# BuzzLord/godot-audio-spatializer

Hardware: AMD Instinct MI355X
Metric: mixed AudioFrames/s (higher is better)
Workload: dtype f32

## Files before the change

godot-audio-spatializer_amd/csrc/k_hrtf_multi.hip:

```cpp
#include "gas_hrtf_wave.h"

namespace {

constexpr int MW = 8;
constexpr int MAXB = GAS_HRTF_MULTI_MAX_BLOCKS;

template <int SQ>
struct MultiLds {
	static constexpr int SLICES_F2 = MW * LDS_F2_HALF;
	static constexpr int FD_F2 = MW * 2 * 512;
	static constexpr int TOTAL_F2 = SLICES_F2 + FD_F2;
	static constexpr int HL = (8 - SQ) * 64;
	static constexpr int LEFT_BYTES = 160 * 1024 - TOTAL_F2 * 8 - 1024 * 8 - 64;
	static constexpr int HIST_ROWS = LEFT_BYTES / (MW * HL * 4);
};

__device__ __forceinline__ void lds_wait_at_least(const uint32_t *flag, uint32_t want) {
	while (__atomic_load_n(flag, __ATOMIC_RELAXED) < want) {
		__builtin_amdgcn_s_sleep(1);
	}
	__builtin_amdgcn_fence(__ATOMIC_ACQUIRE, "workgroup");
}

template <int SQ, bool HIST_LDS>
__global__ __launch_bounds__(MW * 64, GAS_HRTF_WAVES_PER_SIMD) void k_hrtf_multi(gas_group_args g, gas_hrtf_blocks mb, const uint32_t *__restrict__ peak_bits, uint32_t peak_all, gas_dev_state st, gas_hrtf_table tab, const float2 *__restrict__ tw, float *__restrict__ partials) {
	constexpr int FQ = 2 * SQ;
	constexpr int HQ = 8 - SQ;
	constexpr int NQ = 8 + SQ;
	constexpr uint32_t F = FQ * 64;
	constexpr uint32_t HL = HQ * 64;
	__shared__ float2 lds_all[MultiLds<SQ>::TOTAL_F2];
	__shared__ float2 tw_lds[1024];
	__shared__ float hist_lds[HIST_LDS ? MW * MultiLds<SQ>::HIST_ROWS * HL : 4];
	__shared__ uint32_t arrived, consumed;
	const int lane = threadIdx.x & 63;
	const int wave = __builtin_amdgcn_readfirstlane(threadIdx.x >> 6);
	float2 *lds = lds_all + wave * LDS_F2_HALF;
	float *my_hist = hist_lds + (HIST_LDS ? wave * MultiLds<SQ>::HIST_ROWS * HL : 0);
	float2 *fd = lds_all + MultiLds<SQ>::SLICES_F2;
	const uint32_t K = mb.k;

	const float4 tw_in = reinterpret_cast<const float4 *>(tw)[threadIdx.x & 511];
	if (threadIdx.x == 0) {
		arrived = 0;
		consumed = 0;
	}
	uint32_t first, last;
	wave_range(g.n, blockIdx.x * MW + wave, gridDim.x * MW, first, last);
	const uint32_t cnt = last - first;
	const bool have = (uint32_t)lane < cnt;
	uint32_t my_slot = 0, my_row = 0, my_dir = 0, my_flag = 0;
	float my_g0 = 0.0f, my_g1 = 0.0f;
	if (have) {
		const uint32_t e = first + lane;
		my_slot = g.slots ? g.slots[e] : g.slot_base + e;
		my_row = g.rows ? g.rows[e] : e;
	}
	gas_audio_frame raw[FQ];
	float rawh[HQ];
	if (cnt > 0) {
		const uint32_t s0 = (uint32_t)__builtin_amdgcn_readlane((int)my_slot, 0), r0 = (uint32_t)__builtin_amdgcn_readlane((int)my_row, 0);
		if constexpr (HIST_LDS) {
			constexpr int HR = MultiLds<SQ>::HIST_ROWS;
			float stage[HR][HQ];
#pragma unroll
			for (int r = 0; r < HR; r++) {
				if ((uint32_t)r < cnt) {
					const uint32_t sr = (uint32_t)__builtin_amdgcn_readlane((int)my_slot, r);
					load_history<HQ>(st.hrtf_hist + (size_t)sr * HL, lane, stage[r]);
				}
			}
#pragma unroll
			for (int r = 0; r < HR; r++) {
				if ((uint32_t)r < cnt) {
					store_history<HQ>(my_hist + (size_t)r * HL, lane, stage[r]);
				}
			}
		} else {
			load_history<HQ>(st.hrtf_hist + (size_t)s0 * HL, lane, rawh);
		}
#pragma unroll
		for (int q = 0; q < FQ; q++) {
			raw[q] = (GAS_ABL & 8) ? gas_audio_frame{ (float)lane, (float)r0 } : nt_load_frame(mb.src[0] + (size_t)r0 * F + lane + 64 * q);
		}
	}
	auto block_params = [&](uint32_t b, float keep_g, uint32_t keep_d, float &g1, uint32_t &d) {
		const gas_params *fr = mb.fresh[b];
		g1 = keep_g;
		d = keep_d;
		if (have && (fr || b == 0)) {
			const gas_params *P = fr ? fr + my_row : st.params + my_slot;
			const float2 gd = *reinterpret_cast<const float2 *>(&P->hrtf_gain);
			const uint32_t dd = __float_as_uint(gd.y);
			g1 = gd.x;
			d = dd < tab.dirs ? dd : 0;
		}
	};
	if (have) {
		my_g0 = st.hrtf_prev_gain[my_slot];
		const uint32_t e = first + lane;
		my_flag = peak_all ? 1u : (peak_bits ? (peak_bits[e >> 5] >> (e & 31)) & 1u : 0u);
	}
	block_params(0, 0.0f, 0, my_g1, my_dir);
	if (threadIdx.x < 512) {
		reinterpret_cast<float4 *>(tw_lds)[threadIdx.x] = tw_in;
	}
	__syncthreads();
	float2 t1[8], t2[8];
#pragma unroll
	for (int k = 0; k < 8; k++) {
		t1[k] = tw_lds[k * 64 + lane];
		t2[k] = tw_lds[(8 + k) * 64 + lane];
	}
	const float lane_f = (float)lane;

	for (uint32_t b = 0; b < K; b++) {
		float *peaks_b = mb.peaks[b];
		const gas_audio_frame *src_b = mb.src[b];
		const gas_audio_frame *src_wrap = mb.src[b + 1 < K ? b + 1 : b];
		float2 aYL[8], aYR[8], zp[8];
		float4 hs[8];
#pragma unroll
		for (int j = 0; j < 8; j++) {
			aYL[j] = make_float2(0.0f, 0.0f);
			aYR[j] = make_float2(0.0f, 0.0f);
			zp[j] = make_float2(0.0f, 0.0f);
		}
		float nx_g1 = my_g1;
		uint32_t nx_dir = my_dir;
		if (b + 1 < K) {
			block_params(b + 1, my_g1, my_dir, nx_g1, nx_dir);
		}
		bool have_prev = false;
		uint32_t prev_flag = 0, prev_row = 0;
		auto products = [&](bool more, uint32_t next_dir) {
			float2 yl[8], yr[8];
			if (have_prev) {
				finish_spectra(lane, hs);
#pragma unroll
				for (int j = 0; j < 8; j++) {
					cmac_fixed(aYL[j], zp[j], hs[j].x, hs[j].y);
					cmac_fixed(aYR[j], zp[j], hs[j].z, hs[j].w);
				}
				if (prev_flag) {
#pragma unroll
					for (int j = 0; j < 8; j++) {
						yl[j] = cmul_fixed(zp[j], hs[j].x, hs[j].y);
						yr[j] = cmul_fixed(zp[j], hs[j].z, hs[j].w);
					}
				}
			}
			if (more) {
				issue_spectra(tab.spec, next_dir, lane, hs);
			}
			if (have_prev && prev_flag) {
				fft512<true>(yl, t1, t2, lds, lane);
				fft512<true>(yr, t1, t2, lds, lane);
				float pkl = 0.0f, pkr = 0.0f;
#pragma unroll
				for (int t = 0; t < SQ; t++) {
					pkl = fmaxf(pkl, fmaxf(fabsf(yl[HQ + t].x), fabsf(yl[HQ + t].y)));
					pkr = fmaxf(pkr, fmaxf(fabsf(yr[HQ + t].x), fabsf(yr[HQ + t].y)));
				}
				pkl = wave_max(pkl);
				pkr = wave_max(pkr);
				if (lane == 0) {
					peaks_b[(size_t)prev_row * 2] = pkl;
					peaks_b[(size_t)prev_row * 2 + 1] = pkr;
				}
			}
		};

		for (uint32_t i = 0; i < cnt; i++) {
			const uint32_t slot = (uint32_t)__builtin_amdgcn_readlane((int)my_slot, (int)i);
			const uint32_t row = (uint32_t)__builtin_amdgcn_readlane((int)my_row, (int)i);
			const uint32_t dir = (uint32_t)__builtin_amdgcn_readlane((int)my_dir, (int)i);
			const float g0 = __int_as_float(__builtin_amdgcn_readlane(__float_as_int(my_g0), (int)i));
			const float g1 = __int_as_float(__builtin_amdgcn_readlane(__float_as_int(my_g1), (int)i));
			const uint32_t flag = (uint32_t)__builtin_amdgcn_readlane((int)my_flag, (int)i);
			float xq[NQ];
			if constexpr (HIST_LDS) {
				load_history<HQ>(my_hist + (size_t)i * HL, lane, rawh);
			}
#pragma unroll
			for (int q = 0; q < HQ; q++) {
				xq[q] = rawh[q];
			}
			if constexpr (!HIST_LDS) {
#pragma unroll
				for (int q = 0; q < hrtf_dead_regs<SQ>(); q++) {
					asm volatile("" ::"v"(rawh[q]));
				}
			}
			float lf = lane_f;
			asm volatile("" : "+v"(lf));
#pragma unroll
			for (int q = 0; q < hrtf_unkept_regs<SQ>(); q++) {
				const float mono = (raw[q].left + raw[q].right) * 0.5f;
				const float t = (lf + (float)(64 * q)) * (1.0f / (float)F);
				xq[HQ + q] = window_sample(mono, ramp_weight(g0, g1, t, 1 - t));
			}
#pragma unroll
			for (int q = hrtf_unkept_regs<SQ>(); q < FQ; q++) {
				const float mono = (raw[q].left + raw[q].right) * 0.5f;
				const float t = (lf + (float)(64 * q)) * (1.0f / (float)F);
				xq[HQ + q] = window_sample_kept(mono, ramp_weight(g0, g1, t, 1 - t));
			}
			if (!HIST_LDS || b + 1 == K) {
				store_history<HQ>(st.hrtf_hist + (size_t)slot * HL, lane, &xq[FQ]);
			} else {
				store_history<HQ>(my_hist + (size_t)i * HL, lane, &xq[FQ]);
			}
			const bool wrap = i + 1 == cnt;
			{
				const uint32_t ni = wrap ? 0u : i + 1;
				const uint32_t nrow = (uint32_t)__builtin_amdgcn_readlane((int)my_row, (int)ni);
				const gas_audio_frame *nsrc = (wrap ? src_wrap : src_b) + (size_t)nrow * F;
				if constexpr (!HIST_LDS) {
					const uint32_t nslot = (uint32_t)__builtin_amdgcn_readlane((int)my_slot, (int)ni);
					load_history<HQ>(st.hrtf_hist + (size_t)nslot * HL, lane, rawh);
				}
#pragma unroll
				for (int q = 0; q < FQ; q++) {
					raw[q] = (GAS_ABL & 8) ? gas_audio_frame{ (float)lane, (float)nrow } : nt_load_frame(nsrc + lane + 64 * q);
				}
			}
			float2 zs[8];
#pragma unroll
			for (int j = 0; j < 8; j++) {
				zs[j] = hrtf_window_z<SQ>(xq, j);
			}
			fft512<false>(zs, t1, t2, lds, lane);
			products(true, dir);
#pragma unroll
			for (int j = 0; j < 8; j++) {
				zp[j] = zs[j];
			}
			have_prev = true;
			prev_flag = flag;
			prev_row = row;
		}
		const int ep0 = (int)(2 * (b & 3));
		const gas_deferred_reduce job = mb.job[b];
		float4 jr[JOB_ROWS];
		const uint32_t jw = (uint32_t)((wave - ep0 - 2) & 7), jx = blockIdx.x & 7, ji = blockIdx.x >> 3;
		const uint32_t job_col = (((ji >> 1) * 8 + jx) * 8) + (ji & 1) * 4 + jw;
		const bool job_mine = job.partials != nullptr && jw < GAS_HRTF_JOB_WAVES && job_col < job.elems / 4;
		products(false, 0);

		lds_wait_at_least(&consumed, 2 * b);
#pragma unroll
		for (int j = 0; j < 8; j++) {
			fd[(wave * 2 + 0) * 512 + j * 64 + lane] = aYL[j];
			fd[(wave * 2 + 1) * 512 + j * 64 + lane] = aYR[j];
		}
		__builtin_amdgcn_fence(__ATOMIC_RELEASE, "workgroup");
		if (lane == 0) {
			__atomic_fetch_add(&arrived, 1u, __ATOMIC_RELAXED);
		}
		if (job_mine) {
			job_issue(job, job_col, lane, jr);
			job_finish(job, job_col, lane, jr);
		}
		if (wave == ep0 || wave == ep0 + 1) {
			const int ear = wave - ep0;
			lds_wait_at_least(&arrived, MW * (b + 1));
			float2 y[8];
#pragma unroll
			for (int j = 0; j < 8; j++) {
				y[j] = fd[ear * 512 + j * 64 + lane];
			}
#pragma unroll
			for (int w = 1; w < MW; w++) {
#pragma unroll
				for (int j = 0; j < 8; j++) {
					y[j] = cadd(y[j], fd[(w * 2 + ear) * 512 + j * 64 + lane]);
				}
			}
			__builtin_amdgcn_fence(__ATOMIC_RELEASE, "workgroup");
			if (lane == 0) {
				__atomic_fetch_add(&consumed, 1u, __ATOMIC_RELAXED);
			}
			fft512<true>(y, t1, t2, lds, lane);
			float *my_partial = partials + ((size_t)mb.p_offset[b] + blockIdx.x) * (size_t)(F * 2);
#pragma unroll
			for (int t = 0; t < SQ; t++) {
				const int fa = lane + 64 * t, fb = lane + 64 * (SQ + t);
				my_partial[fa * 2 + ear] = y[HQ + t].x;
				my_partial[fb * 2 + ear] = y[HQ + t].y;
			}
		}
		if (have && !my_flag) {
			*reinterpret_cast<float2 *>(peaks_b + (size_t)my_row * 2) = make_float2(__builtin_inff(), __builtin_inff());
		}
		my_g0 = my_g1;
		my_g1 = nx_g1;
		my_dir = nx_dir;
	}

	if (have) {
		st.hrtf_prev_gain[my_slot] = my_g0;
		if (mb.last_fresh) {
			const float4 *src4 = reinterpret_cast<const float4 *>(mb.last_fresh + my_row);
			float4 *dst4 = reinterpret_cast<float4 *>(st.params + my_slot);
#pragma unroll
			for (int k = 0; k < 8; k++) {
				dst4[k] = src4[k];
			}
		}
	}
}

}

bool gas_hrtf_multi_hist_in_lds(uint32_t n, uint32_t frames) {
	const uint32_t wgs = gas_hrtf_uni_partials(n);
	const uint32_t per_wave = (n + wgs * MW - 1) / (wgs * MW);
	switch (frames / 128) {
		case 1:
			return per_wave <= (uint32_t)MultiLds<1>::HIST_ROWS;
		case 2:
			return per_wave <= (uint32_t)MultiLds<2>::HIST_ROWS;
		case 3:
			return per_wave <= (uint32_t)MultiLds<3>::HIST_ROWS;
		default:
			return per_wave <= (uint32_t)MultiLds<4>::HIST_ROWS;
	}
}

hipError_t gas_launch_hrtf_multi(hipStream_t stream, const gas_group_args &g, const gas_hrtf_blocks &mb, const uint32_t *peak_bits, bool peak_all, const gas_dev_state &st, const gas_hrtf_table &tab, const float2 *twiddles, uint32_t frames, uint32_t hist_len, float *partials) {
	if (g.n == 0 || mb.k == 0) {
		return hipSuccess;
	}
	const uint32_t wgs = gas_hrtf_uni_partials(g.n);
	if (frames % 128 != 0 || frames > 512 || hist_len != 512 - frames / 2 || g.order != nullptr || mb.k > (uint32_t)MAXB || g.n < wgs * MW || g.n > wgs * MW * 64 || gas_hrtf_uni_waves() != (uint32_t)MW) {
		return hipErrorInvalidValue;
	}
	dim3 grid(wgs), block(MW * 64);
	const uint32_t all = peak_all ? 1u : 0u;
	const uint32_t per_wave = (g.n + wgs * MW - 1) / (wgs * MW);
#define GAS_MULTI_CASE(SQv)                                                                                                                     \
	case SQv:                                                                                                                                   \
		if (per_wave <= (uint32_t)MultiLds<SQv>::HIST_ROWS) {                                                                                   \
			hipLaunchKernelGGL((k_hrtf_multi<SQv, true>), grid, block, 0, stream, g, mb, peak_bits, all, st, tab, twiddles, partials);          \
		} else {                                                                                                                                \
			hipLaunchKernelGGL((k_hrtf_multi<SQv, false>), grid, block, 0, stream, g, mb, peak_bits, all, st, tab, twiddles, partials);         \
		}                                                                                                                                       \
		break;
	switch (frames / 128) {
		GAS_MULTI_CASE(1)
		GAS_MULTI_CASE(2)
		GAS_MULTI_CASE(3)
		GAS_MULTI_CASE(4)
		default:
			return hipErrorInvalidValue;
	}
#undef GAS_MULTI_CASE
	return hipGetLastError();
}
```

Baseline: 401.2 billion.

## Process pairs of blocks per source when parameters are unchanged, reusing spectra

When the next block has no fresh parameters, two consecutive blocks are handled together per source. The HRTF spectra for the direction are fetched once and applied to both blocks' FFTs, and the second block's window reuses history kept in registers. To save registers it reads twiddles from LDS (fft512_twlds) instead of holding them, and the epilogue is factored into a shared lambda. This cuts spectra loads and history round-trips but adds LDS twiddle traffic and register pressure from four accumulator sets.

```diff
diff --git a/godot-audio-spatializer_amd/csrc/k_hrtf_multi.hip b/godot-audio-spatializer_amd/csrc/k_hrtf_multi.hip
--- a/godot-audio-spatializer_amd/csrc/k_hrtf_multi.hip
+++ b/godot-audio-spatializer_amd/csrc/k_hrtf_multi.hip
@@ -1,4 +1,6 @@
 #include "gas_hrtf_wave.h"
+
+#include <type_traits>
 
 namespace {
 
@@ -22,6 +24,11 @@
 	__builtin_amdgcn_fence(__ATOMIC_ACQUIRE, "workgroup");
 }
 
+__device__ __forceinline__ int opaque_lane(int l) {
+	asm volatile("" : "+v"(l));
+	return l;
+}
+
 template <int SQ, bool HIST_LDS>
 __global__ __launch_bounds__(MW * 64, GAS_HRTF_WAVES_PER_SIMD) void k_hrtf_multi(gas_group_args g, gas_hrtf_blocks mb, const uint32_t *__restrict__ peak_bits, uint32_t peak_all, gas_dev_state st, gas_hrtf_table tab, const float2 *__restrict__ tw, float *__restrict__ partials) {
 	constexpr int FQ = 2 * SQ;
@@ -29,6 +36,7 @@
 	constexpr int NQ = 8 + SQ;
 	constexpr uint32_t F = FQ * 64;
 	constexpr uint32_t HL = HQ * 64;
+	constexpr bool PAIRS = HIST_LDS || SQ <= 2;
 	__shared__ float2 lds_all[MultiLds<SQ>::TOTAL_F2];
 	__shared__ float2 tw_lds[1024];
 	__shared__ float hist_lds[HIST_LDS ? MW * MultiLds<SQ>::HIST_ROWS * HL : 4];
@@ -48,6 +56,7 @@
 	uint32_t first, last;
 	wave_range(g.n, blockIdx.x * MW + wave, gridDim.x * MW, first, last);
 	const uint32_t cnt = last - first;
+	__builtin_assume(cnt > 0);
 	const bool have = (uint32_t)lane < cnt;
 	uint32_t my_slot = 0, my_row = 0, my_dir = 0, my_flag = 0;
 	float my_g0 = 0.0f, my_g1 = 0.0f;
@@ -73,7 +82,7 @@
 #pragma unroll
 			for (int r = 0; r < HR; r++) {
 				if ((uint32_t)r < cnt) {
-					store_history<HQ>(my_hist + (size_t)r * HL, lane, stage[r]);
+					store_history<HQ>(my_hist + (size_t)r * HL, opaque_lane(lane), stage[r]);
 				}
 			}
 		} else {
@@ -89,7 +98,9 @@
 		g1 = keep_g;
 		d = keep_d;
 		if (have && (fr || b == 0)) {
-			const gas_params *P = fr ? fr + my_row : st.params + my_slot;
+			uint32_t pr = my_row, ps = my_slot;
+			asm volatile("" : "+v"(pr), "+v"(ps));
+			const gas_params *P = fr ? fr + pr : st.params + ps;
 			const float2 gd = *reinterpret_cast<const float2 *>(&P->hrtf_gain);
 			const uint32_t dd = __float_as_uint(gd.y);
 			g1 = gd.x;
@@ -107,14 +118,250 @@
 	}
 	__syncthreads();
 	float2 t1[8], t2[8];
-#pragma unroll
-	for (int k = 0; k < 8; k++) {
-		t1[k] = tw_lds[k * 64 + lane];
-		t2[k] = tw_lds[(8 + k) * 64 + lane];
-	}
 	const float lane_f = (float)lane;
 
-	for (uint32_t b = 0; b < K; b++) {
+	auto window = [&](float (&xq)[NQ], float g0, float g1) {
+		float lf = lane_f;
+		asm volatile("" : "+v"(lf));
+#pragma unroll
+		for (int q = 0; q < hrtf_unkept_regs<SQ>(); q++) {
+			const float mono = (raw[q].left + raw[q].right) * 0.5f;
+			const float t = (lf + (float)(64 * q)) * (1.0f / (float)F);
+			xq[HQ + q] = window_sample(mono, ramp_weight(g0, g1, t, 1 - t));
+		}
+#pragma unroll
+		for (int q = hrtf_unkept_regs<SQ>(); q < FQ; q++) {
+			const float mono = (raw[q].left + raw[q].right) * 0.5f;
+			const float t = (lf + (float)(64 * q)) * (1.0f / (float)F);
+			xq[HQ + q] = window_sample_kept(mono, ramp_weight(g0, g1, t, 1 - t));
+		}
+	};
+	auto block_duties = [&](auto in_pair, uint32_t b, const float2 (&aYL)[8], const float2 (&aYR)[8], float *peaks_b) {
+		const int ep0 = (int)(2 * (b & 3));
+		const gas_deferred_reduce job = mb.job[b];
+		float4 jr[JOB_ROWS];
+		const uint32_t jw = (uint32_t)((wave - ep0 - 2) & 7), jx = blockIdx.x & 7, ji = blockIdx.x >> 3;
+		const uint32_t job_col = (((ji >> 1) * 8 + jx) * 8) + (ji & 1) * 4 + jw;
+		const bool job_mine = job.partials != nullptr && jw < GAS_HRTF_JOB_WAVES && job_col < job.elems / 4;
+
+		lds_wait_at_least(&consumed, 2 * b);
+		const int fl = opaque_lane(lane);
+#pragma unroll
+		for (int j = 0; j < 8; j++) {
+			fd[(wave * 2 + 0) * 512 + j * 64 + fl] = aYL[j];
+			fd[(wave * 2 + 1) * 512 + j * 64 + fl] = aYR[j];
+		}
+		__builtin_amdgcn_fence(__ATOMIC_RELEASE, "workgroup");
+		if (lane == 0) {
+			__atomic_fetch_add(&arrived, 1u, __ATOMIC_RELAXED);
+		}
+		if (job_mine) {
+			job_issue(job, job_col, lane, jr);
+			job_finish(job, job_col, lane, jr);
+		}
+		if (wave == ep0 || wave == ep0 + 1) {
+			const int ear = wave - ep0;
+			lds_wait_at_least(&arrived, MW * (b + 1));
+			float2 y[8];
+#pragma unroll
+			for (int j = 0; j < 8; j++) {
+				y[j] = fd[ear * 512 + j * 64 + fl];
+			}
+#pragma unroll
+			for (int w = 1; w < MW; w++) {
+#pragma unroll
+				for (int j = 0; j < 8; j++) {
+					y[j] = cadd(y[j], fd[(w * 2 + ear) * 512 + j * 64 + fl]);
+				}
+			}
+			__builtin_amdgcn_fence(__ATOMIC_RELEASE, "workgroup");
+			if (lane == 0) {
+				__atomic_fetch_add(&consumed, 1u, __ATOMIC_RELAXED);
+			}
+			if constexpr (decltype(in_pair)::value) {
+				fft512_twlds<true>(y, tw_lds, lds, lane);
+			} else {
+				fft512<true>(y, t1, t2, lds, lane);
+			}
+			float *my_partial = partials + ((size_t)mb.p_offset[b] + blockIdx.x) * (size_t)(F * 2);
+#pragma unroll
+			for (int t = 0; t < SQ; t++) {
+				const int fa = lane + 64 * t, fb = lane + 64 * (SQ + t);
+				my_partial[fa * 2 + ear] = y[HQ + t].x;
+				my_partial[fb * 2 + ear] = y[HQ + t].y;
+			}
+		}
+		if (have && !my_flag) {
+			float inf = __builtin_inff();
+			asm volatile("" : "+v"(inf));
+			*reinterpret_cast<float2 *>(peaks_b + (size_t)my_row * 2) = make_float2(inf, inf);
+		}
+	};
+
+	for (uint32_t next_b = 0;;) {
+		const uint32_t b = (uint32_t)__builtin_amdgcn_readfirstlane((int)next_b);
+		if (b >= K) {
+			break;
+		}
+		if (PAIRS && b + 1 < K && mb.fresh[b + 1] == nullptr) {
+			float *peaks_0 = mb.peaks[b], *peaks_1 = mb.peaks[b + 1];
+			const gas_audio_frame *src_0 = mb.src[b], *src_1 = mb.src[b + 1];
+			const gas_audio_frame *src_wrap = mb.src[b + 2 < K ? b + 2 : b + 1];
+			const bool writes_back = b + 2 == K;
+			float2 aL0[8], aR0[8], aL1[8], aR1[8];
+			float4 hs[8];
+#pragma unroll
+			for (int j = 0; j < 8; j++) {
+				aL0[j] = make_float2(0.0f, 0.0f);
+				aR0[j] = make_float2(0.0f, 0.0f);
+				aL1[j] = make_float2(0.0f, 0.0f);
+				aR1[j] = make_float2(0.0f, 0.0f);
+			}
+			float nx_g1 = my_g1;
+			uint32_t nx_dir = my_dir;
+			if (b + 2 < K) {
+				block_params(b + 2, my_g1, my_dir, nx_g1, nx_dir);
+			}
+			auto exact_peak = [&](const float2 (&z)[8], float *peaks_b, uint32_t row) {
+				float pk[2];
+#pragma unroll
+				for (int ear = 0; ear < 2; ear++) {
+					float2 y[8];
+#pragma unroll
+					for (int j = 0; j < 8; j++) {
+						y[j] = ear == 0 ? cmul_fixed(z[j], hs[j].x, hs[j].y) : cmul_fixed(z[j], hs[j].z, hs[j].w);
+					}
+					fft512_twlds<true>(y, tw_lds, lds, lane);
+					float p = 0.0f;
+#pragma unroll
+					for (int t = 0; t < SQ; t++) {
+						p = fmaxf(p, fmaxf(fabsf(y[HQ + t].x), fabsf(y[HQ + t].y)));
+					}
+					pk[ear] = wave_max(p);
+				}
+				if (lane == 0) {
+					peaks_b[(size_t)row * 2] = pk[0];
+					peaks_b[(size_t)row * 2 + 1] = pk[1];
+				}
+			};
+			issue_spectra(tab.spec, (uint32_t)__builtin_amdgcn_readlane((int)my_dir, 0), lane, hs);
+			float keep[HQ];
+			auto first_half = [&](uint32_t i) {
+				const uint32_t row = (uint32_t)__builtin_amdgcn_readlane((int)my_row, (int)i);
+				const float g0 = __int_as_float(__builtin_amdgcn_readlane(__float_as_int(my_g0), (int)i));
+				const float g1 = __int_as_float(__builtin_amdgcn_readlane(__float_as_int(my_g1), (int)i));
+				const uint32_t flag = (uint32_t)__builtin_amdgcn_readlane((int)my_flag, (int)i);
+				float xq[NQ];
+				if constexpr (HIST_LDS) {
+					load_history<HQ>(my_hist + (size_t)i * HL, opaque_lane(lane), rawh);
+				}
+#pragma unroll
+				for (int q = 0; q < HQ; q++) {
+					xq[q] = rawh[q];
+				}
+				if constexpr (!HIST_LDS) {
+#pragma unroll
+					for (int q = 0; q < hrtf_dead_regs<SQ>(); q++) {
+						asm volatile("" ::"v"(rawh[q]));
+					}
+				}
+				window(xq, g0, g1);
+#pragma unroll
+				for (int q = 0; q < HQ; q++) {
+					keep[q] = xq[FQ + q];
+				}
+#pragma unroll
+				for (int q = 0; q < FQ; q++) {
+					raw[q] = (GAS_ABL & 8) ? gas_audio_frame{ (float)lane, (float)row } : nt_load_frame(src_1 + (size_t)row * F + lane + 64 * q);
+				}
+				float2 zs[8];
+#pragma unroll
+				for (int j = 0; j < 8; j++) {
+					zs[j] = hrtf_window_z<SQ>(xq, j);
+				}
+				fft512_twlds<false>(zs, tw_lds, lds, lane);
+				finish_spectra(lane, hs);
+#pragma unroll
+				for (int j = 0; j < 8; j++) {
+					cmac_fixed(aL0[j], zs[j], hs[j].x, hs[j].y);
+					cmac_fixed(aR0[j], zs[j], hs[j].z, hs[j].w);
+				}
+				if (flag) {
+					exact_peak(zs, peaks_0, row);
+				}
+			};
+			auto second_half = [&](uint32_t i, bool wrap) {
+				const uint32_t slot = (uint32_t)__builtin_amdgcn_readlane((int)my_slot, (int)i);
+				const uint32_t row = (uint32_t)__builtin_amdgcn_readlane((int)my_row, (int)i);
+				const float g1 = __int_as_float(__builtin_amdgcn_readlane(__float_as_int(my_g1), (int)i));
+				const uint32_t flag = (uint32_t)__builtin_amdgcn_readlane((int)my_flag, (int)i);
+				float xr[NQ];
+#pragma unroll
+				for (int q = 0; q < HQ; q++) {
+					xr[q] = keep[q];
+				}
+				window(xr, g1, g1);
+				if (!HIST_LDS || writes_back) {
+					store_history<HQ>(st.hrtf_hist + (size_t)slot * HL, lane, &xr[FQ]);
+				} else {
+					store_history<HQ>(my_hist + (size_t)i * HL, opaque_lane(lane), &xr[FQ]);
+				}
+				const uint32_t ni = wrap ? 0u : i + 1;
+				const uint32_t nrow = (uint32_t)__builtin_amdgcn_readlane((int)my_row, (int)ni);
+				const gas_audio_frame *nsrc = (wrap ? src_wrap : src_0) + (size_t)nrow * F;
+				if constexpr (!HIST_LDS) {
+					const uint32_t nslot = (uint32_t)__builtin_amdgcn_readlane((int)my_slot, (int)ni);
+					load_history<HQ>(st.hrtf_hist + (size_t)nslot * HL, lane, rawh);
+				}
+#pragma unroll
+				for (int q = 0; q < FQ; q++) {
+					raw[q] = (GAS_ABL & 8) ? gas_audio_frame{ (float)lane, (float)nrow } : nt_load_frame(nsrc + lane + 64 * q);
+				}
+				float2 zs[8];
+#pragma unroll
+				for (int j = 0; j < 8; j++) {
+					zs[j] = hrtf_window_z<SQ>(xr, j);
+				}
+				fft512_twlds<false>(zs, tw_lds, lds, lane);
+#pragma unroll
+				for (int j = 0; j < 8; j++) {
+					cmac_fixed(aL1[j], zs[j], hs[j].x, hs[j].y);
+					cmac_fixed(aR1[j], zs[j], hs[j].z, hs[j].w);
+				}
+				if (flag) {
+					exact_peak(zs, peaks_1, row);
+				}
+				issue_spectra(tab.spec, (uint32_t)__builtin_amdgcn_readlane((int)my_dir, (int)ni), lane, hs);
+			};
+			for (uint32_t i = 0;; i++) {
+				first_half(i);
+				if (i + 1 >= cnt) {
+					break;
+				}
+				second_half(i, false);
+			}
+#pragma unroll
+			for (int q = 0; q < FQ; q++) {
+				asm volatile("" : "+v"(raw[q].left), "+v"(raw[q].right));
+			}
+			block_duties(std::true_type{}, b, aL0, aR0, peaks_0);
+			second_half(cnt - 1, true);
+			block_duties(std::true_type{}, b + 1, aL1, aR1, peaks_1);
+			my_g0 = my_g1;
+			my_g1 = nx_g1;
+			my_dir = nx_dir;
+			next_b = b + 2;
+			continue;
+		}
+		{
+			int l = lane;
+			asm volatile("" : "+v"(l));
+#pragma unroll
+			for (int k = 0; k < 8; k++) {
+				t1[k] = tw_lds[k * 64 + l];
+				t2[k] = tw_lds[(8 + k) * 64 + l];
+			}
+		}
 		float *peaks_b = mb.peaks[b];
 		const gas_audio_frame *src_b = mb.src[b];
 		const gas_audio_frame *src_wrap = mb.src[b + 1 < K ? b + 1 : b];
@@ -125,6 +372,7 @@
 			aYL[j] = make_float2(0.0f, 0.0f);
 			aYR[j] = make_float2(0.0f, 0.0f);
 			zp[j] = make_float2(0.0f, 0.0f);
+			hs[j] = make_float4(0.0f, 0.0f, 0.0f, 0.0f);
 		}
 		float nx_g1 = my_g1;
 		uint32_t nx_dir = my_dir;
@@ -180,7 +428,7 @@
 			const uint32_t flag = (uint32_t)__builtin_amdgcn_readlane((int)my_flag, (int)i);
 			float xq[NQ];
 			if constexpr (HIST_LDS) {
-				load_history<HQ>(my_hist + (size_t)i * HL, lane, rawh);
+				load_history<HQ>(my_hist + (size_t)i * HL, opaque_lane(lane), rawh);
 			}
 #pragma unroll
 			for (int q = 0; q < HQ; q++) {
@@ -192,24 +440,11 @@
 					asm volatile("" ::"v"(rawh[q]));
 				}
 			}
-			float lf = lane_f;
-			asm volatile("" : "+v"(lf));
-#pragma unroll
-			for (int q = 0; q < hrtf_unkept_regs<SQ>(); q++) {
-				const float mono = (raw[q].left + raw[q].right) * 0.5f;
-				const float t = (lf + (float)(64 * q)) * (1.0f / (float)F);
-				xq[HQ + q] = window_sample(mono, ramp_weight(g0, g1, t, 1 - t));
-			}
-#pragma unroll
-			for (int q = hrtf_unkept_regs<SQ>(); q < FQ; q++) {
-				const float mono = (raw[q].left + raw[q].right) * 0.5f;
-				const float t = (lf + (float)(64 * q)) * (1.0f / (float)F);
-				xq[HQ + q] = window_sample_kept(mono, ramp_weight(g0, g1, t, 1 - t));
-			}
+			window(xq, g0, g1);
 			if (!HIST_LDS || b + 1 == K) {
 				store_history<HQ>(st.hrtf_hist + (size_t)slot * HL, lane, &xq[FQ]);
 			} else {
-				store_history<HQ>(my_hist + (size_t)i * HL, lane, &xq[FQ]);
+				store_history<HQ>(my_hist + (size_t)i * HL, opaque_lane(lane), &xq[FQ]);
 			}
 			const bool wrap = i + 1 == cnt;
 			{
@@ -240,62 +475,12 @@
 			prev_flag = flag;
 			prev_row = row;
 		}
-		const int ep0 = (int)(2 * (b & 3));
-		const gas_deferred_reduce job = mb.job[b];
-		float4 jr[JOB_ROWS];
-		const uint32_t jw = (uint32_t)((wave - ep0 - 2) & 7), jx = blockIdx.x & 7, ji = blockIdx.x >> 3;
-		const uint32_t job_col = (((ji >> 1) * 8 + jx) * 8) + (ji & 1) * 4 + jw;
-		const bool job_mine = job.partials != nullptr && jw < GAS_HRTF_JOB_WAVES && job_col < job.elems / 4;
 		products(false, 0);
-
-		lds_wait_at_least(&consumed, 2 * b);
-#pragma unroll
-		for (int j = 0; j < 8; j++) {
-			fd[(wave * 2 + 0) * 512 + j * 64 + lane] = aYL[j];
-			fd[(wave * 2 + 1) * 512 + j * 64 + lane] = aYR[j];
-		}
-		__builtin_amdgcn_fence(__ATOMIC_RELEASE, "workgroup");
-		if (lane == 0) {
-			__atomic_fetch_add(&arrived, 1u, __ATOMIC_RELAXED);
-		}
-		if (job_mine) {
-			job_issue(job, job_col, lane, jr);
-			job_finish(job, job_col, lane, jr);
-		}
-		if (wave == ep0 || wave == ep0 + 1) {
-			const int ear = wave - ep0;
-			lds_wait_at_least(&arrived, MW * (b + 1));
-			float2 y[8];
-#pragma unroll
-			for (int j = 0; j < 8; j++) {
-				y[j] = fd[ear * 512 + j * 64 + lane];
-			}
-#pragma unroll
-			for (int w = 1; w < MW; w++) {
-#pragma unroll
-				for (int j = 0; j < 8; j++) {
-					y[j] = cadd(y[j], fd[(w * 2 + ear) * 512 + j * 64 + lane]);
-				}
-			}
-			__builtin_amdgcn_fence(__ATOMIC_RELEASE, "workgroup");
-			if (lane == 0) {
-				__atomic_fetch_add(&consumed, 1u, __ATOMIC_RELAXED);
-			}
-			fft512<true>(y, t1, t2, lds, lane);
-			float *my_partial = partials + ((size_t)mb.p_offset[b] + blockIdx.x) * (size_t)(F * 2);
-#pragma unroll
-			for (int t = 0; t < SQ; t++) {
-				const int fa = lane + 64 * t, fb = lane + 64 * (SQ + t);
-				my_partial[fa * 2 + ear] = y[HQ + t].x;
-				my_partial[fb * 2 + ear] = y[HQ + t].y;
-			}
-		}
-		if (have && !my_flag) {
-			*reinterpret_cast<float2 *>(peaks_b + (size_t)my_row * 2) = make_float2(__builtin_inff(), __builtin_inff());
-		}
+		block_duties(std::false_type{}, b, aYL, aYR, peaks_b);
 		my_g0 = my_g1;
 		my_g1 = nx_g1;
 		my_dir = nx_dir;
+		next_b = b + 1;
 	}
 
 	if (have) {
```

Result: no change. 402.4 billion, median of 2 (+0.3%).
